# nubot-nudt/RDMNet

Hardware: AMD Instinct MI355X
Metric: scan-pairs/sec (whole node) (higher is better)
Workload: dtype f32

## Files before the change

include/rdmnet_hip.h:

```cpp
#ifndef RDMNET_HIP_H_
#define RDMNET_HIP_H_

#include <stddef.h>
#include <stdint.h>

#ifdef __cplusplus
extern "C" {
#endif

#define RDM_ABI_VERSION 2

int rdm_abi_version(void);
size_t rdm_abi_struct_size(int which);
const char* rdm_last_error(void);

int rdm_rehash_schedule(int64_t max_elems, int64_t* at_host, int64_t* buckets_host, int cap);

size_t rdm_grid_subsample_workspace_bytes(int64_t n_points, int batch);
int rdm_grid_subsample(const float* points, int64_t n_points, const int64_t* lengths, int batch,
                       float voxel_size, float* out_points, int64_t* out_lengths, void* ws,
                       size_t ws_bytes, void* stream);
int rdm_grid_subsample_form(const float* points, int64_t n_points, const int64_t* lengths, int batch, float voxel_size,
                            float* out_points, int64_t* out_lengths, void* ws, size_t ws_bytes, void* stream, int form);

// ... 157 lines not shown
int rdm_row_positive(const float* x, int64_t n, int64_t c, int64_t ld, uint8_t* out, void* stream);

size_t rdm_group_norm_workspace_bytes(int64_t n, int64_t c);
int rdm_group_norm(const float* x, int64_t n, int64_t c, int64_t ldx, int groups, const float* gamma,
                   const float* beta, float eps, const float* residual, int64_t ldr, int act, float* y,
                   int64_t ldy, uint8_t* positive, void* ws, size_t ws_bytes, void* stream);
int rdm_group_norm_form(const float* x, int64_t n, int64_t c, int64_t ldx, int groups, const float* gamma,
                        const float* beta, float eps, const float* residual, int64_t ldr, int act, float* y, int64_t ldy,
                        uint8_t* positive, void* ws, size_t ws_bytes, int form, void* stream);
size_t rdm_linear_group_norm_workspace_bytes(int64_t m, int64_t n);
int rdm_linear_group_norm(const float* x, int64_t ldx, const float* w, int64_t ldw, const float* bias,
                          const float* rowdiv, int64_t m, int64_t n, int64_t k, int groups, const float* gamma,
                          const float* beta, float eps, const float* residual, int64_t ldr, int act, float* lin_out,
                          int64_t ld_lin, float* y, int64_t ldy, uint8_t* positive, void* ws, size_t ws_bytes,
                          void* stream);
int rdm_patch_scores(const float* ref_feats, int64_t ld_ref, int64_t n_ref, const int64_t* ref_idx, const float* src_feats,
                     int64_t ld_src, int64_t n_src, const int64_t* src_idx, int64_t batch, int64_t side, int64_t d,
                     const float* rowdiv, float* scores, void* stream);
size_t rdm_decoder_stage_workspace_bytes(int64_t m, int64_t n, int64_t k);
int rdm_decoder_stage(const float* coarse, int64_t n_coarse, int64_t c1, int64_t ld1, const int64_t* idx, int64_t ldi,
                      const float* skip, int64_t c2, int64_t ld2, int64_t m, const float* w, int64_t ldw, const float* bias,
                      int64_t n, int groups, const float* gamma, const float* beta, float eps, int act, float* lin_out,
                      int64_t ld_lin, float* y, int64_t ldy, void* ws, size_t ws_bytes, void* stream);
int rdm_layer_norm(const float* x, int64_t n, int64_t c, int64_t ldx, const float* residual,
                   int64_t ldr, const float* gamma, const float* beta, float eps, int act, float* y,
                   int64_t ldy, void* stream);
int rdm_linear_layer_norm(const float* x, int64_t ldx, const float* w, int64_t ldw, const float* bias, int64_t m, int64_t n,
                          int64_t k, const float* residual, int64_t ldr, const float* gamma, const float* beta, float eps,
                          int act, float* y, int64_t ldy, void* stream);
int rdm_attention_tail(const float* hidden, int64_t ld_hidden, const float* x, int64_t ldx, int64_t m, int64_t d,
// ... 372 lines not shown
```

rdmnet_amd/_lib.py:

```python
import ctypes
import os

_HERE = os.path.dirname(os.path.abspath(__file__))
LIB_PATH = os.environ.get('RDM_LIB_PATH') or os.path.join(_HERE, 'librdmnet_hip.so')

c_void = ctypes.c_void_p
c_i64 = ctypes.c_int64
c_int = ctypes.c_int
c_f32 = ctypes.c_float
c_size = ctypes.c_size_t

ABI_VERSION = 2


class FineMatchingOptions(ctypes.Structure):
    _fields_ = [('topk', ctypes.c_int32), ('mutual', ctypes.c_int32), ('use_dustbin', ctypes.c_int32),
                ('use_global_score', ctypes.c_int32), ('confidence_threshold', ctypes.c_float),
                ('correspondence_limit', ctypes.c_int32)]

    @classmethod
    def of(cls, topk=1, mutual=False, use_dustbin=True, confidence_threshold=0.0, use_global_score=False,
           correspondence_limit=None):
        return cls(int(topk), int(bool(mutual)), int(bool(use_dustbin)), int(bool(use_global_score)), float(confidence_threshold),
                   0 if correspondence_limit is None else int(correspondence_limit))
# ... 124 lines not shown
    'rdm_pose_graph_pair_covariances_host': (c_int, [c_i64, c_i64, c_void, c_void, c_void, c_i64, c_void, c_void]),
    'rdm_pose_graph_pair_terms_host': (c_int, [c_void, c_void, c_void, c_void, c_void, c_void, c_void, c_void]),
    'rdm_pose_graph_edge_terms_host': (c_int, [c_void, c_void, c_void, c_void, ctypes.c_double, c_int, c_void]),
    'rdm_pose_graph_retract_host': (c_int, [c_void, c_void, c_void]),
    'rdm_neighbor_histogram': (c_int, [c_void, c_i64, c_void, c_int, c_void]),
    'rdm_radius_grid_records': (c_void, [c_void, c_size, c_i64]),
    'rdm_row_positive': (c_int, [c_void, c_i64, c_i64, c_i64, c_void, c_void]),
    'rdm_group_norm_workspace_bytes': (c_size, [c_i64, c_i64]),
    'rdm_group_norm': (c_int, [c_void, c_i64, c_i64, c_i64, c_int, c_void, c_void, c_f32, c_void, c_i64, c_int,
                               c_void, c_i64, c_void, c_void, c_size, c_void]),
    'rdm_group_norm_form': (c_int, [c_void, c_i64, c_i64, c_i64, c_int, c_void, c_void, c_f32, c_void, c_i64, c_int,
                                    c_void, c_i64, c_void, c_void, c_size, c_int, c_void]),
    'rdm_linear_group_norm_workspace_bytes': (c_size, [c_i64, c_i64]),
    'rdm_linear_group_norm': (c_int, [c_void, c_i64, c_void, c_i64, c_void, c_void, c_i64, c_i64, c_i64, c_int, c_void, c_void,
                                      c_f32, c_void, c_i64, c_int, c_void, c_i64, c_void, c_i64, c_void, c_void, c_size, c_void]),
    'rdm_patch_scores': (c_int, [c_void, c_i64, c_i64, c_void, c_void, c_i64, c_i64, c_void, c_i64, c_i64, c_i64, c_void, c_void,
                                 c_void]),
    'rdm_decoder_stage_workspace_bytes': (c_size, [c_i64, c_i64, c_i64]),
    'rdm_decoder_stage': (c_int, [c_void, c_i64, c_i64, c_i64, c_void, c_i64, c_void, c_i64, c_i64, c_i64, c_void, c_i64, c_void,
                                  c_i64, c_int, c_void, c_void, c_f32, c_int, c_void, c_i64, c_void, c_i64, c_void, c_size, c_void]),
    'rdm_layer_norm': (c_int, [c_void, c_i64, c_i64, c_i64, c_void, c_i64, c_void, c_void, c_f32, c_int, c_void,
                               c_i64, c_void]),
    'rdm_linear_layer_norm': (c_int, [c_void, c_i64, c_void, c_i64, c_void, c_i64, c_i64, c_i64, c_void, c_i64, c_void, c_void,
                                      c_f32, c_int, c_void, c_i64, c_void]),
    'rdm_attention_tail': (c_int, [c_void, c_i64, c_void, c_i64, c_i64, c_i64, c_void, c_i64, c_void, c_void, c_void, c_void, c_i64,
                                   c_void, c_void, c_i64, c_void, c_void, c_void, c_f32, c_void, c_i64, c_void]),
    'rdm_attention_tail_packed_floats': (c_size, []),
    'rdm_attention_tail_pack_weights': (c_int, [c_void, c_i64, c_void, c_i64, c_void, c_i64, c_void, c_void]),
    'rdm_attention_tail_packed': (c_int, [c_void, c_i64, c_void, c_i64, c_i64, c_i64, c_void, c_void, c_void, c_void, c_void, c_void,
                                          c_void, c_void, c_f32, c_void, c_i64, c_void]),
# ... 198 lines not shown
```

rdmnet_amd/csrc/engine.hip:

```cpp
#include <algorithm>
#include <cmath>
#include <cstring>
#include <atomic>
#include <chrono>
#include <functional>
#include <map>
#include <memory>
#include <string>
#include <vector>

#include "../../include/rdmnet_hip.h"
#include <ctime>

#include "common.h"
#include "internal.h"
#include "lockstep.h"

namespace {

using namespace rdm;

struct Mat {
  float* p = nullptr;
  int64_t rows = 0, cols = 0, ld = 0;
// ... 226 lines not shown
  lockstep_align();
  rdm_engine* e = r.e;
  const Linear* Lp = lin_param(r, name + ".mlp");
  if (!Lp) return RDM_ERR_ARG;
  const Linear& L = *Lp;
  Mat t = e->mat(x.rows, L.out);
  y = e->mat(x.rows, L.out);
  ENG_ALLOC(t.p); ENG_ALLOC(y.p);
  float *g, *b;
  ENG_CHECK(norm_params(r, name + ".norm.norm", &g, &b));
  return rdm_linear_group_norm(x.p, x.ld, L.b, L.ldb, L.bias, nullptr, x.rows, L.out, L.kpad, r.groups, g, b, 1e-5f,
                               res ? res->p : nullptr, res ? res->ld : 0, act, t.p, t.ld, y.p, y.ld, positive, r.ws,
                               r.ws_bytes, r.st);
}

int decoder_stage(Run& r, const std::string& lin_name, const std::string* norm_name, const Mat& coarse, const int64_t* up_idx,
                  int64_t up_ld, const Mat& skip, int64_t m, Mat& y, int64_t n_cols = 0) {
  lockstep_align();
  rdm_engine* e = r.e;
  const Linear* Lp = lin_param(r, lin_name);
  if (!Lp) return RDM_ERR_ARG;
  const Linear& L = *Lp;
  RDM_REQUIRE(coarse.cols + skip.cols == L.in, "rdm_engine: %s expects %lld input columns", lin_name.c_str(), (long long)L.in);
  RDM_REQUIRE(n_cols >= 0 && n_cols <= L.out && (n_cols == 0 || !norm_name), "rdm_engine: %s cannot compute %lld of its columns",
              lin_name.c_str(), (long long)n_cols);
  const int64_t n = n_cols > 0 ? n_cols : L.out;
  Mat t = e->mat(m, L.out);
  ENG_ALLOC(t.p);
  float *g = nullptr, *b = nullptr;
  if (norm_name) {
// ... 1111 lines not shown
      ENG_CHECK(kpconv(rr, name + ".KPConv", x, enc.x_pos, q, s, t, sigma, name + ".norm", y, order));
    } else {
      Mat h = x;
      uint8_t* h_pos = e->alloc<uint8_t>(x.rows > 0 ? x.rows : 1);
      ENG_ALLOC(h_pos);
      if (e->params->lin.count(name + ".unary1.mlp")) {
        ENG_CHECK(unary(rr, name + ".unary1", x, h, 2, nullptr, h_pos));
      } else {
        ENG_CHECK(rdm_row_positive(x.p, x.rows, x.cols, x.ld, h_pos, rr.st));
      }
      Mat cn;
      Mat sc = x;
      ENG_CHECK(kpconv(rr, name + ".KPConv", h, h_pos, q, s, t, sigma, name + ".norm_conv", cn, order,
                       strided[b] ? &x : nullptr, strided[b] ? &sc : nullptr));
      if (e->params->lin.count(name + ".unary_shortcut.mlp")) {
        Mat s2;
        ENG_CHECK(unary(rr, name + ".unary_shortcut", sc, s2, 0, nullptr, nullptr));
        sc = s2;
      }
      ENG_CHECK(unary(rr, name + ".unary2", cn, y, 2, &sc, nullptr));
    }
    x = y;
    tap(rr, name.c_str(), x);
    if (b % 3 == 1) enc.feats[b / 3] = x;
  }
  enc.blocks = b1;
  return RDM_OK;
}

struct Coarse {
  Mat buf;
  Mat x;
  float* n2p = nullptr;
};

// ... 385 lines not shown
  const rdm_engine_config& c = e->cfg;
  const int64_t n0 = n_ref + n_src;
  Level* lv = py.lv;
  py.flags = e->alloc<int32_t>(64);
  ENG_ALLOC(py.flags);
  bool overlap_l0 = false;
  if (overlap) {
    const auto t_poll = std::chrono::steady_clock::now();
    do {
      overlap_l0 = hipStreamQuery(r.st) == hipSuccess;
    } while (!overlap_l0 && std::chrono::steady_clock::now() - t_poll < std::chrono::microseconds(40));
  }
  Run rs = r;
  if (overlap_l0) {
    rs.st = e->side;
    rs.ws_bytes = std::max<size_t>(size_t(96) << 20, rdm_linear_group_norm_workspace_bytes(n0, 128));
    rs.ws = e->alloc<char>(rs.ws_bytes);
    ENG_ALLOC(rs.ws);
  }
  fill_words<int32_t>(py.flags, 64, 0, overlap_l0 ? rs.st : r.st);
  const bool full = e->keep_taps || e->collate_only;
  lv[0].n = n0; lv[0].n_ref = n_ref;
  lv[0].pts = e->alloc<float>(3 * n0);
  lv[0].lengths = e->alloc<int64_t>(2);
  ENG_ALLOC(lv[0].pts); ENG_ALLOC(lv[0].lengths);
  float* pts0 = lv[0].pts;
  int64_t* len0 = lv[0].lengths;
  if (overlap_l0) {
    pts0 = e->alloc<float>(3 * n0);
    len0 = e->alloc<int64_t>(2);
    ENG_ALLOC(pts0); ENG_ALLOC(len0);
// ... 87 lines not shown
  else if (dd) ENG_CHECK(pyramid_from_data_dict(r, *dd, py));
  else ENG_CHECK(collate_pair(r, overlap, side_guard, ref_points, n_ref, src_points, n_src, py, enc));
  for (int i = 0; i < 5; ++i) {
    res->level_sizes[i] = py.lv[i].n;
    res->level_ref_sizes[i] = py.lv[i].n_ref;
  }
  tap_pyramid(r, py);
  if (e->collate_only) {
    res->arena_used = e->arena_off;
    return RDM_OK;
  }

  {
    size_t need = r.ws_bytes;
    for (int l = 0; l < c.num_stages; ++l)
      need = std::max(need, rdm_linear_group_norm_workspace_bytes(py.lv[l].n, int64_t(128) << l));
    if (need > r.ws_bytes) {
      r.ws_bytes = need;
      r.ws = e->alloc<char>(r.ws_bytes);
      ENG_ALLOC(r.ws);
    }
  }

  if (enc.blocks == 0) ENG_CHECK(encoder_input(r, dd, n0, enc));
  ENG_CHECK(encoder_blocks(r, py, enc.blocks, 14, enc));
  tap(r, "feats_c_enc", enc.feats[4]);
  Coarse co;
  ENG_CHECK(transformer1(r, py, enc.feats[4], co));

  Mat dec;
  const std::function<int()> fork_decoder = [&]() -> int {
// ... 379 lines not shown
```

rdmnet_amd/csrc/gemm.hip:

```cpp
#include "../../include/rdmnet_hip.h"
#include <cmath>
#include <cstdlib>

#include "common.h"
#include "internal.h"
#include "lockstep.h"

namespace {

using namespace rdm;

typedef float f32x16 __attribute__((ext_vector_type(16)));
typedef float f32x4_t __attribute__((ext_vector_type(4)));

struct GemmArgs {
  const float* A = nullptr;
  const float* B = nullptr;
  float* C = nullptr;
  const float* bias = nullptr;
  const float* rowdiv = nullptr;
  int M = 0, N = 0, K = 0;
  int lda = 0, ldb = 0, ldc = 0;
  long long sa = 0, sb = 0, sc = 0;
  int act = 0;
// ... 1113 lines not shown
  char* gws = ar.take<char>(gemm_ws);
  double* partial = ar.take<double>(static_cast<size_t>(gemm_stats_max_blocks(m)) * 2 * n);
  const size_t gn_ws = rdm_group_norm_workspace_bytes(m, n);
  char* nws = ar.take<char>(gn_ws);
  if (!ar.ok) {
    set_error("rdm_linear_group_norm: workspace too small (%zu < %zu)", ws_bytes, ar.off);
    return RDM_ERR_WORKSPACE;
  }
  int nblk = 0;
  if (int e = gemm_with_stats(x, ldx, w, ldw, lin_out, ld_lin, m, n, k, bias, rowdiv, gws, gemm_ws, partial, &nblk, stream))
    return e;
  return group_norm_finish(partial, nblk, lin_out, m, n, ld_lin, groups, gamma, beta, eps, residual, ldr, act, y, ldy,
                           positive, nws, gn_ws, stream);
}

extern "C" int rdm_patch_scores(const float* ref_feats, int64_t ld_ref, int64_t n_ref, const int64_t* ref_idx,
                                const float* src_feats, int64_t ld_src, int64_t n_src, const int64_t* src_idx, int64_t batch,
                                int64_t side, int64_t d, const float* rowdiv, float* scores, void* stream) {
  using namespace rdm;
  RDM_REQUIRE(ref_feats && src_feats && ref_idx && src_idx && scores, "rdm_patch_scores: null pointer");
  RDM_REQUIRE(batch >= 0 && side > 0 && d > 0 && d % 4 == 0 && ld_ref % 4 == 0 && ld_src % 4 == 0 && n_ref > 0 && n_src > 0,
              "rdm_patch_scores: bad sizes");
  RDM_REQUIRE(((reinterpret_cast<uintptr_t>(ref_feats) | reinterpret_cast<uintptr_t>(src_feats)) & 15) == 0,
              "rdm_patch_scores: features must be 16-byte aligned");
  if (batch == 0) return RDM_OK;
  GemmArgs g;
  g.A = ref_feats; g.B = src_feats; g.C = scores; g.rowdiv = rowdiv;
  g.M = static_cast<int>(side); g.N = static_cast<int>(side); g.K = static_cast<int>(d);
  g.lda = static_cast<int>(ld_ref); g.ldb = static_cast<int>(ld_src); g.ldc = static_cast<int>(side);
  g.sc = side * side;
// ... 135 lines not shown
```

rdmnet_amd/csrc/internal.h:

```cpp
#pragma once
#include <cstddef>
#include <cstdint>

namespace rdm {

int gemm_with_stats(const float* a, int64_t lda, const float* b, int64_t ldb, float* c, int64_t ldc, int64_t m,
                    int64_t n, int64_t k, const float* bias, const float* rowdiv, void* ws, size_t ws_bytes,
                    double* gn_partial, int* gn_blocks, void* stream);

void gemm_set_lds_pad(unsigned bytes);
int gemm_concat_with_stats(const float* coarse, int64_t ld1, int64_t c1, int64_t n_coarse, const int64_t* idx, int64_t ldi,
                           const float* skip, int64_t ld2, int64_t c2, const float* b, int64_t ldb, float* c, int64_t ldc,
                           int64_t m, int64_t n, int64_t n_need, const float* bias, int act, float* pbuf, size_t pbuf_floats,
                           void* ws, size_t ws_bytes, double* gn_partial, int* gn_blocks, void* stream);
int decoder_stage_cols(const float* coarse, int64_t n_coarse, int64_t c1, int64_t ld1, const int64_t* idx, int64_t ldi,
                       const float* skip, int64_t c2, int64_t ld2, int64_t m, const float* w, int64_t ldw, const float* bias,
                       int64_t n, int64_t n_need, int groups, const float* gamma, const float* beta, float eps, int act,
                       float* lin_out, int64_t ld_lin, float* y, int64_t ldy, void* ws, size_t ws_bytes, void* stream);

int gemm_pair(const float* a0, int64_t lda0, const float* b0, int64_t ldb0, float* c0, int64_t ldc0, int64_t m0, int64_t n0,
              int64_t k0, const float* bias0, const float* a1, int64_t lda1, const float* b1, int64_t ldb1, float* c1,
              int64_t ldc1, int64_t m1, int64_t n1, int64_t k1, const float* bias1, void* ws, size_t ws_bytes, void* stream);

inline int64_t gemm_stats_max_blocks(int64_t m) { return (m + 7) / 8 + 1; }

int grid_subsample_mode(const float* points, int64_t n_points, const int64_t* lengths, int batch, float voxel_size,
                        float* out_points, int64_t* out_lengths, void* ws, size_t ws_bytes, void* stream, int mode);

int group_norm_finish(const double* partial, int nblk, const float* x, int64_t n, int64_t c, int64_t ldx, int groups,
                      const float* gamma, const float* beta, float eps, const float* residual, int64_t ldr, int act,
                      float* y, int64_t ldy, uint8_t* positive, void* ws, size_t ws_bytes, void* stream, int form = 0);

int gather_rows_multi(int n, const void* const* x, const int64_t* n_src, const int64_t* words, const int64_t* ldx,
                      const int64_t* const* idx, const int64_t* m, void* const* y, const int64_t* ldy, void* stream);

int radius_grid_build_multi(int n, const float* const* s_points, const int64_t* n_s, const int64_t* const* s_lengths, int batch,
                            const float* radius, void* const* grid_ws, const size_t* grid_ws_bytes, void* stream);

int radius_grid_build_trivial(const float* s_points, int64_t n_s, const int64_t* s_lengths, int batch, void* grid_ws,
                              size_t grid_ws_bytes, void* stream);

int compact_indices_pair(const uint8_t* keep, int64_t n_ref, int64_t n, int32_t* order, int32_t* counts,
                         const int32_t* mirror_src, int32_t* mirror_dst, int mirror_words, void* stream);

int gather_max_ordered(const float* x, int64_t n_s, int64_t c, int64_t ldx, const int64_t* idx, int64_t m, int64_t h, int64_t ldi,
                       const int32_t* width, float* y, int64_t ldy, const float* order_records, int i32, void* stream);
// ... 24 lines not shown
```

rdmnet_amd/csrc/norm.hip:

```cpp
#include "../../include/rdmnet_hip.h"
#include "common.h"
#include "internal.h"
#include "lockstep.h"

namespace {

using namespace rdm;

constexpr int kGnRowsPerBlock = 64;

__device__ __forceinline__ void gn_partial_kernel_body(const dim3 blockIdx, const dim3 gridDim, const float* x, int n, int c, int ld,
                                                         double* partial) {
  (void)blockIdx; (void)gridDim;
  __shared__ double red[2][256];
  const int r0 = blockIdx.x * kGnRowsPerBlock;
  const int r1 = min(n, r0 + kGnRowsPerBlock);
  const int cw = c < 256 ? c : 256;
  const int lanes = 256 / cw;
  const int col_in = threadIdx.x % cw, rl = threadIdx.x / cw;
  const int col = blockIdx.y * 256 + col_in;
  double s = 0.0, ss = 0.0;
  if (rl < lanes && col < c)
    for (int r = r0 + rl; r < r1; r += lanes) {
      const double v = x[static_cast<int64_t>(r) * ld + col];
// ... 88 lines not shown
    for (int blk = 0; blk < nblk; ++blk) {
      a += partial[(static_cast<int64_t>(blk) * 2 + 0) * c + k];
      b += partial[(static_cast<int64_t>(blk) * 2 + 1) * c + k];
    }
    gs += a;
    gss += b;
  }
  const double cnt = static_cast<double>(n) * cpg;
  const double mean = gs / cnt;
  double var = gss / cnt - mean * mean;
  if (var < 0.0) var = 0.0;
  const double gsc = 1.0 / sqrt(var + static_cast<double>(eps)) * static_cast<double>(gamma[col]);
  scale[col] = static_cast<float>(gsc);
  shift[col] = static_cast<float>(static_cast<double>(beta[col]) - mean * gsc);
}
template <int COLS>
__device__ __forceinline__ void gn_finalize_kernel_body(const dim3 blockIdx, const dim3 gridDim, const double* partial, int nblk, int n,
                                                            int c, int groups, const float* gamma,
                                                            const float* beta, float eps, float* scale,
                                                            float* shift) {
  (void)blockIdx; (void)gridDim;
  __shared__ GnFinalizeLds<COLS> L;
  const float2 v = gn_scale_shift<COLS>(L, blockIdx.x * COLS, partial, nblk, n, c, groups, gamma, beta, eps);
  const int col = blockIdx.x * COLS + threadIdx.x % COLS;
  if (threadIdx.x / COLS == 0 && col < c) {
    scale[col] = v.x;
    shift[col] = v.y;
  }
}


constexpr int kGnFusedRows = 256;
__device__ __forceinline__ void gn_finalize_apply_kernel_body(const dim3 blockIdx, const dim3 gridDim, const double* partial, int nblk, const float* x, int n, int c, int ldx,
                                                                  int groups, const float* gamma, const float* beta, float eps,
                                                                  const float* res, int ldr, int act, float* y, int ldy) {
  (void)blockIdx; (void)gridDim;
  __shared__ GnFinalizeLds<64> L;
  __shared__ float sc_l[64], sh_l[64];
  const int col0 = blockIdx.x * 64;
  const float2 v = gn_scale_shift<64>(L, col0, partial, nblk, n, c, groups, gamma, beta, eps);
  if (threadIdx.x < 64) {
    sc_l[threadIdx.x] = v.x;
    sh_l[threadIdx.x] = v.y;
  }
  __syncthreads();
  const int q = threadIdx.x & 15, rl = threadIdx.x >> 4;
  const int col = col0 + 4 * q;
  if (col >= c) return;
  const float4 sc = *reinterpret_cast<const float4*>(sc_l + 4 * q), sh = *reinterpret_cast<const float4*>(sh_l + 4 * q);
  const int r1 = min(n, (static_cast<int>(blockIdx.y) + 1) * kGnFusedRows);
  for (int row = blockIdx.y * kGnFusedRows + rl; row < r1; row += 64) {
    const float4 xv = *reinterpret_cast<const float4*>(x + static_cast<int64_t>(row) * ldx + col);
    float o[4] = {__builtin_fmaf(xv.x, sc.x, sh.x), __builtin_fmaf(xv.y, sc.y, sh.y), __builtin_fmaf(xv.z, sc.z, sh.z),
                  __builtin_fmaf(xv.w, sc.w, sh.w)};
    if (res) {
      const float4 rv = *reinterpret_cast<const float4*>(res + static_cast<int64_t>(row) * ldr + col);
      o[0] += rv.x; o[1] += rv.y; o[2] += rv.z; o[3] += rv.w;
    }
#pragma unroll
    for (int k = 0; k < 4; ++k) {
      if (act == 2) o[k] = o[k] > 0.f ? o[k] : 0.1f * o[k];
      else if (act == 1) o[k] = o[k] > 0.f ? o[k] : 0.f;
    }
    *reinterpret_cast<float4*>(y + static_cast<int64_t>(row) * ldy + col) = make_float4(o[0], o[1], o[2], o[3]);
  }
}


__device__ __forceinline__ void gn_apply_kernel_body(const dim3 blockIdx, const dim3 gridDim, const float* x, int n, int c, int ldx,
                                                       const float* scale, const float* shift,
                                                       const float* res, int ldr, int act, float* y,
                                                       int ldy, unsigned char* positive) {
  (void)blockIdx; (void)gridDim;
  const int row = blockIdx.x * 4 + (threadIdx.x >> 6);
  if (row >= n) return;
  const int lane = threadIdx.x & 63;
  float rs = 0.f;
  for (int col = lane; col < c; col += 64) {
    float v = x[static_cast<int64_t>(row) * ldx + col] * scale[col] + shift[col];
    if (res) v += res[static_cast<int64_t>(row) * ldr + col];
    if (act == 2) v = v > 0.f ? v : 0.1f * v;
    else if (act == 1) v = v > 0.f ? v : 0.f;
    y[static_cast<int64_t>(row) * ldy + col] = v;
    rs += v;
  }
  if (positive) {
    rs = wave_sum(rs);
    if (lane == 0) positive[row] = rs > 0.f ? 1 : 0;
  }
}


__device__ __forceinline__ void gn_apply_wide_kernel_body(const dim3 blockIdx, const dim3 gridDim, const float* x, int n, int c4, int ldx, const float* scale,
                                                            const float* shift, const float* res, int ldr, int act,
                                                            float* y, int ldy, unsigned char* positive) {
  (void)blockIdx; (void)gridDim;
  const int64_t t = blockIdx.x * 256ll + threadIdx.x;
  const bool live = t < static_cast<int64_t>(n) * c4;
  if (!live && !positive) return;
  float rs4[4] = {0.f, 0.f, 0.f, 0.f};
  const int row = live ? static_cast<int>(t / c4) : 0, col = live ? static_cast<int>(t % c4) * 4 : 0;
  if (live) {
  const float4 xv = *reinterpret_cast<const float4*>(x + static_cast<int64_t>(row) * ldx + col);
  const float4 sc = *reinterpret_cast<const float4*>(scale + col), sh = *reinterpret_cast<const float4*>(shift + col);
  float v[4] = {__builtin_fmaf(xv.x, sc.x, sh.x), __builtin_fmaf(xv.y, sc.y, sh.y), __builtin_fmaf(xv.z, sc.z, sh.z),
                __builtin_fmaf(xv.w, sc.w, sh.w)};
  if (res) {
    const float4 rv = *reinterpret_cast<const float4*>(res + static_cast<int64_t>(row) * ldr + col);
    v[0] += rv.x; v[1] += rv.y; v[2] += rv.z; v[3] += rv.w;
  }
#pragma unroll
  for (int k = 0; k < 4; ++k) {
    if (act == 2) v[k] = v[k] > 0.f ? v[k] : 0.1f * v[k];
    else if (act == 1) v[k] = v[k] > 0.f ? v[k] : 0.f;
  }
  *reinterpret_cast<float4*>(y + static_cast<int64_t>(row) * ldy + col) = make_float4(v[0], v[1], v[2], v[3]);
#pragma unroll
  for (int k = 0; k < 4; ++k) rs4[k] = v[k];
  }
  if (positive) {
    for (int o = c4 >> 1; o > 0; o >>= 1)
#pragma unroll
      for (int k = 0; k < 4; ++k) rs4[k] += __shfl_xor(rs4[k], o, 64);
// ... 211 lines not shown
                     static_cast<uint32_t*>(y), static_cast<int>(ldy));
  else if (threads == 128) ::rdm::launch<gather_rows_kernel_body, 128>(dim3(static_cast<unsigned>(m)), 0, static_cast<hipStream_t>(stream), static_cast<const uint32_t*>(x), static_cast<int>(n_src),
                     static_cast<int>(words), static_cast<int>(ldx), idx, static_cast<int>(m),
                     static_cast<uint32_t*>(y), static_cast<int>(ldy));
  else ::rdm::launch<gather_rows_kernel_body, 64>(dim3(static_cast<unsigned>(m)), 0, static_cast<hipStream_t>(stream), static_cast<const uint32_t*>(x), static_cast<int>(n_src),
                     static_cast<int>(words), static_cast<int>(ldx), idx, static_cast<int>(m),
                     static_cast<uint32_t*>(y), static_cast<int>(ldy));
  return launch_status("gather_rows_kernel");
}

extern "C" size_t rdm_group_norm_workspace_bytes(int64_t n, int64_t c) {
  const size_t nblk = static_cast<size_t>(rdm::ceil_div<int64_t>(n > 0 ? n : 1, kGnRowsPerBlock));
  return rdm::align_up(nblk * 2 * c * sizeof(double)) + rdm::align_up(2 * c * sizeof(float));
}

int rdm::group_norm_finish(const double* partial_in, int nblk, const float* x, int64_t n, int64_t c, int64_t ldx,
                           int groups, const float* gamma, const float* beta, float eps, const float* residual,
                           int64_t ldr, int act, float* y, int64_t ldy, uint8_t* positive, void* ws, size_t ws_bytes,
                           void* stream, int form) {
  Arena ar(ws, ws_bytes);
  const int own_blk = static_cast<int>(ceil_div<int64_t>(n, kGnRowsPerBlock));
  double* partial = ar.take<double>(static_cast<size_t>(own_blk) * 2 * c);
  float* ss = ar.take<float>(2 * c);
  if (!ar.ok) {
    set_error("rdm_group_norm: workspace too small (%zu < %zu)", ws_bytes, ar.off);
    return RDM_ERR_WORKSPACE;
  }
  hipStream_t st = static_cast<hipStream_t>(stream);
  const double* use = partial_in;
  if (nblk <= 0) {
    ::rdm::launch<gn_partial_kernel_body, 256>(dim3(own_blk, ceil_div<int64_t>(c, 256)), 0, st, x,
                       static_cast<int>(n), static_cast<int>(c), static_cast<int>(ldx), partial);
    use = partial;
    nblk = own_blk;
  }
  const bool vec_ok = c % 4 == 0 && ldx % 4 == 0 && ldy % 4 == 0 && (!residual || ldr % 4 == 0) &&
                      (reinterpret_cast<uintptr_t>(x) & 15) == 0 && (reinterpret_cast<uintptr_t>(y) & 15) == 0 &&
                      (!residual || (reinterpret_cast<uintptr_t>(residual) & 15) == 0);
  static const bool fin64 = ::rdm::dev_knob("RDM_GN_FINALIZE_64") != nullptr;
  const bool narrow = !fin64 && nblk >= 128 && c / groups <= 16 && 16 % (c / groups) == 0;
  const bool whole_groups = 64 % (c / groups) == 0;
  if (form != 1 && !narrow && !positive && vec_ok && c % 64 == 0 && n <= 4096 && whole_groups) {
    RDM_DUP_LOOP("gnfin")
    ::rdm::launch<gn_finalize_apply_kernel_body, 1024>(dim3(static_cast<unsigned>(c / 64), static_cast<unsigned>(ceil_div<int64_t>(n, kGnFusedRows))), 0, st, use, nblk, x, static_cast<int>(n), static_cast<int>(c), static_cast<int>(ldx), groups, gamma, beta,
                       eps, residual, static_cast<int>(ldr), act, y, static_cast<int>(ldy));
    return launch_status("gn_finalize_apply_kernel");
  }
  {
    RDM_DUP_LOOP("gnfin")
    if (!whole_groups)
      ::rdm::launch<gn_finalize_any_width_kernel_body, 256>(dim3(ceil_div<int64_t>(c, 256)), 0, st, use, nblk,
                         static_cast<int>(n), static_cast<int>(c), groups, gamma, beta, eps, ss, ss + c);
    else if (narrow)
      ::rdm::launch<gn_finalize_kernel_body<16>, 1024>(dim3(ceil_div<int64_t>(c, 16)), 0, st, use, nblk,
                         static_cast<int>(n), static_cast<int>(c), groups, gamma, beta, eps, ss, ss + c);
    else
    ::rdm::launch<gn_finalize_kernel_body<64>, 1024>(dim3(ceil_div<int64_t>(c, 64)), 0, st, use, nblk,
                       static_cast<int>(n), static_cast<int>(c), groups, gamma, beta, eps, ss, ss + c);
  }
  static const bool narrow_rows = ::rdm::dev_knob("RDM_GN_APPLY_ROWS") != nullptr;
  const int64_t c4 = c / 4;
  const bool flag_ok = c4 == 8 || c4 == 16 || c4 == 32;
  const bool wide = vec_ok && (narrow_rows ? (!positive && c >= 256) : (!positive || flag_ok));
  RDM_DUP_LOOP("gnapply")
  if (wide)
    ::rdm::launch<gn_apply_wide_kernel_body, 256>(dim3(ceil_div<int64_t>(n * (c / 4), 256)), 0, st, x, static_cast<int>(n),
                       static_cast<int>(c / 4), static_cast<int>(ldx), ss, ss + c, residual, static_cast<int>(ldr), act, y,
                       static_cast<int>(ldy), positive);
  else
    ::rdm::launch<gn_apply_kernel_body, 256>(dim3(ceil_div<int64_t>(n, 4)), 0, st, x,
                       static_cast<int>(n), static_cast<int>(c), static_cast<int>(ldx), ss, ss + c, residual,
                       static_cast<int>(ldr), act, y, static_cast<int>(ldy), positive);
  return launch_status("group_norm kernels");
}

extern "C" int rdm_group_norm(const float* x, int64_t n, int64_t c, int64_t ldx, int groups,
                              const float* gamma, const float* beta, float eps, const float* residual,
                              int64_t ldr, int act, float* y, int64_t ldy, uint8_t* positive, void* ws,
                              size_t ws_bytes, void* stream) {
  using namespace rdm;
  RDM_REQUIRE(x && gamma && beta && y, "rdm_group_norm: null pointer");
  RDM_REQUIRE(n >= 0 && c > 0 && groups > 0 && c % groups == 0 && c <= 4096 && 64 % (c / groups) == 0,
              "rdm_group_norm: bad sizes (n=%lld c=%lld groups=%d)", (long long)n, (long long)c, groups);
  if (n == 0) return RDM_OK;
  return group_norm_finish(nullptr, 0, x, n, c, ldx, groups, gamma, beta, eps, residual, ldr, act, y, ldy, positive, ws,
                           ws_bytes, stream);
}

// ... 106 lines not shown
```

rdmnet_amd/ops.py:

```python
import ctypes
import numbers

import torch

from . import _lib, config

ACT_NONE, ACT_RELU, ACT_LEAKY = 0, 1, 2


def pad4(n):
    return (int(n) + 3) // 4 * 4


class Scratch:

    def __init__(self, device):
        self.device = device
        self.buf = torch.empty(1 << 24, dtype=torch.uint8, device=device)

    def get(self, nbytes):
        if self.buf.numel() < nbytes:
            self.buf = torch.empty(int(nbytes * 1.25) + 256, dtype=torch.uint8, device=self.device)
        return self.buf

# ... 141 lines not shown

def linear_group_norm(x, b, k, n, bias, gamma, beta, groups, *, rowdiv=None, act=ACT_NONE, residual=None,
                      want_positive=False, eps=1e-5):
    L = _lib.lib()
    m = x.shape[0]
    lin = feat_empty(m, n, x.device)
    y = feat_empty(m, n, x.device)
    pos = torch.empty((max(m, 1),), dtype=torch.uint8, device=x.device) if want_positive else None
    ws = scratch(x.device, L.rdm_linear_group_norm_workspace_bytes(m, n))
    _lib.check(L.rdm_linear_group_norm(x.data_ptr(), _ld(x), b.data_ptr(), _ld(b), _lib.ptr(bias), _lib.ptr(rowdiv), m, n, k,
                                       groups, gamma.data_ptr(), beta.data_ptr(), eps, _lib.ptr(residual),
                                       _ld(residual) if residual is not None else 0, act, lin.data_ptr(), _ld(lin),
                                       y.data_ptr(), _ld(y), _lib.ptr(pos), ws.data_ptr(), ws.numel(), _lib.stream_ptr()),
               'rdm_linear_group_norm')
    return (y, pos) if want_positive else y


def decoder_stage(coarse, idx, skip, b, n, bias, gamma=None, beta=None, groups=32, *, act=ACT_NONE, eps=1e-5):
    L = _lib.lib()
    m, c1, c2 = skip.shape[0], coarse.shape[1], skip.shape[1]
    lin = feat_empty(m, n, skip.device)
    y = feat_empty(m, n, skip.device) if gamma is not None else None
    ws = scratch(skip.device, L.rdm_decoder_stage_workspace_bytes(m, n, c1 + c2))
    _lib.check(L.rdm_decoder_stage(coarse.data_ptr(), coarse.shape[0], c1, _ld(coarse), idx.data_ptr(), _ld(idx), skip.data_ptr(),
                                   c2, _ld(skip), m, b.data_ptr(), _ld(b), _lib.ptr(bias), n, groups, _lib.ptr(gamma),
                                   _lib.ptr(beta), eps, act, lin.data_ptr(), _ld(lin), _lib.ptr(y), _ld(y) if y is not None else 0,
                                   ws.data_ptr(), ws.numel(), _lib.stream_ptr()), 'rdm_decoder_stage')
    return y if gamma is not None else lin


# ... 1867 lines not shown
```

Before: 625.1.

## Fuse shortcut unary group-norm into the residual block's final group-norm apply

In strided residual blocks, the shortcut unary (linear + group norm) used to be run as its own pass and its output then added as the residual of unary2. Now both GEMMs emit partial statistics, and one finalize/apply pass normalises the shortcut product on the fly while adding it to unary2's normalised output. Finalize kernels take a second stat set through blockIdx.y. This removes a separate group-norm finalize and apply pass plus one full write and read of the intermediate, at the cost of extra branching and a larger workspace.

```diff
diff --git a/include/rdmnet_hip.h b/include/rdmnet_hip.h
--- a/include/rdmnet_hip.h
+++ b/include/rdmnet_hip.h
@@ -195,6 +195,12 @@
                           const float* beta, float eps, const float* residual, int64_t ldr, int act, float* lin_out,
                           int64_t ld_lin, float* y, int64_t ldy, uint8_t* positive, void* ws, size_t ws_bytes,
                           void* stream);
+size_t rdm_linear_group_norm_pair_workspace_bytes(int64_t m, int64_t n);
+int rdm_linear_group_norm_pair(const float* x, int64_t ldx, const float* w, int64_t ldw, const float* bias, int64_t k,
+                               const float* xs, int64_t ldxs, const float* w_s, int64_t ldws, const float* bias_s, int64_t ks,
+                               int64_t m, int64_t n, int groups, const float* gamma, const float* beta, const float* gamma_s,
+                               const float* beta_s, float eps, int act, float* lin_out, int64_t ld_lin, float* lin_out_s,
+                               int64_t ld_lin_s, float* y, int64_t ldy, void* ws, size_t ws_bytes, void* stream);
 int rdm_patch_scores(const float* ref_feats, int64_t ld_ref, int64_t n_ref, const int64_t* ref_idx, const float* src_feats,
                      int64_t ld_src, int64_t n_src, const int64_t* src_idx, int64_t batch, int64_t side, int64_t d,
                      const float* rowdiv, float* scores, void* stream);
diff --git a/rdmnet_amd/_lib.py b/rdmnet_amd/_lib.py
--- a/rdmnet_amd/_lib.py
+++ b/rdmnet_amd/_lib.py
@@ -162,6 +162,10 @@
     'rdm_linear_group_norm_workspace_bytes': (c_size, [c_i64, c_i64]),
     'rdm_linear_group_norm': (c_int, [c_void, c_i64, c_void, c_i64, c_void, c_void, c_i64, c_i64, c_i64, c_int, c_void, c_void,
                                       c_f32, c_void, c_i64, c_int, c_void, c_i64, c_void, c_i64, c_void, c_void, c_size, c_void]),
+    'rdm_linear_group_norm_pair_workspace_bytes': (c_size, [c_i64, c_i64]),
+    'rdm_linear_group_norm_pair': (c_int, [c_void, c_i64, c_void, c_i64, c_void, c_i64, c_void, c_i64, c_void, c_i64, c_void, c_i64,
+                                           c_i64, c_i64, c_int, c_void, c_void, c_void, c_void, c_f32, c_int, c_void, c_i64, c_void,
+                                           c_i64, c_void, c_i64, c_void, c_size, c_void]),
     'rdm_patch_scores': (c_int, [c_void, c_i64, c_i64, c_void, c_void, c_i64, c_i64, c_void, c_i64, c_i64, c_i64, c_void, c_void,
                                  c_void]),
     'rdm_decoder_stage_workspace_bytes': (c_size, [c_i64, c_i64, c_i64]),
diff --git a/rdmnet_amd/csrc/engine.hip b/rdmnet_amd/csrc/engine.hip
--- a/rdmnet_amd/csrc/engine.hip
+++ b/rdmnet_amd/csrc/engine.hip
@@ -264,6 +264,39 @@
                                r.ws_bytes, r.st);
 }
 
+int unary_with_shortcut(Run& r, const std::string& name, const Mat& x, const std::string& sc_name, const Mat& sc, Mat& y) {
+  lockstep_align();
+  rdm_engine* e = r.e;
+  const Linear* Lp = lin_param(r, name + ".mlp");
+  const Linear* Sp = Lp ? lin_param(r, sc_name + ".mlp") : nullptr;
+  if (!Lp || !Sp) return RDM_ERR_ARG;
+  const Linear &L = *Lp, &S = *Sp;
+  RDM_REQUIRE(L.out == S.out && x.rows == sc.rows, "rdm_engine: %s and %s disagree in shape", name.c_str(), sc_name.c_str());
+  const int64_t m = x.rows, n = L.out;
+  Mat t = e->mat(m, n), ts = e->mat(m, n);
+  y = e->mat(m, n);
+  ENG_ALLOC(t.p); ENG_ALLOC(ts.p); ENG_ALLOC(y.p);
+  float *g, *b, *gs, *bs;
+  ENG_CHECK(norm_params(r, name + ".norm.norm", &g, &b));
+  ENG_CHECK(norm_params(r, sc_name + ".norm.norm", &gs, &bs));
+  if (m == 0) return RDM_OK;
+  const size_t gemm_ws = rdm_gemm_workspace_bytes(m, n, 1);
+  const size_t stat_bytes = align_up(static_cast<size_t>(gemm_stats_max_blocks(m)) * 2 * n * sizeof(double));
+  const size_t gn_ws = group_norm_residual_norm_workspace_bytes(m, n);
+  RDM_REQUIRE(gemm_ws + 2 * stat_bytes + gn_ws <= r.ws_bytes, "rdm_engine: scratch too small");
+  char* base = static_cast<char*>(r.ws);
+  double* part = reinterpret_cast<double*>(base + gemm_ws);
+  double* part_s = reinterpret_cast<double*>(base + gemm_ws + stat_bytes);
+  int nblk = 0, nblk_s = 0;
+  ENG_CHECK(gemm_with_stats(sc.p, sc.ld, S.b, S.ldb, ts.p, ts.ld, m, n, S.kpad, S.bias, nullptr, r.ws, gemm_ws, part_s, &nblk_s, r.st));
+  lockstep_align();
+  ENG_CHECK(gemm_with_stats(x.p, x.ld, L.b, L.ldb, t.p, t.ld, m, n, L.kpad, L.bias, nullptr, r.ws, gemm_ws, part, &nblk, r.st));
+  lockstep_align();
+  const GnResidualNorm rn{part_s, nblk_s, gs, bs};
+  return group_norm_finish_residual_norm(part, nblk, t.p, m, n, t.ld, r.groups, g, b, 1e-5f, ts.p, ts.ld, rn, 2, y.p, y.ld,
+                                         base + gemm_ws + 2 * stat_bytes, gn_ws, r.st);
+}
+
 int decoder_stage(Run& r, const std::string& lin_name, const std::string* norm_name, const Mat& coarse, const int64_t* up_idx,
                   int64_t up_ld, const Mat& skip, int64_t m, Mat& y, int64_t n_cols = 0) {
   lockstep_align();
@@ -1405,11 +1438,10 @@
       ENG_CHECK(kpconv(rr, name + ".KPConv", h, h_pos, q, s, t, sigma, name + ".norm_conv", cn, order,
                        strided[b] ? &x : nullptr, strided[b] ? &sc : nullptr));
       if (e->params->lin.count(name + ".unary_shortcut.mlp")) {
-        Mat s2;
-        ENG_CHECK(unary(rr, name + ".unary_shortcut", sc, s2, 0, nullptr, nullptr));
-        sc = s2;
+        ENG_CHECK(unary_with_shortcut(rr, name + ".unary2", cn, name + ".unary_shortcut", sc, y));
+      } else {
+        ENG_CHECK(unary(rr, name + ".unary2", cn, y, 2, &sc, nullptr));
       }
-      ENG_CHECK(unary(rr, name + ".unary2", cn, y, 2, &sc, nullptr));
     }
     x = y;
     tap(rr, name.c_str(), x);
@@ -1825,7 +1857,7 @@
   Run rs = r;
   if (overlap_l0) {
     rs.st = e->side;
-    rs.ws_bytes = std::max<size_t>(size_t(96) << 20, rdm_linear_group_norm_workspace_bytes(n0, 128));
+    rs.ws_bytes = std::max<size_t>(size_t(96) << 20, rdm_linear_group_norm_pair_workspace_bytes(n0, 128));
     rs.ws = e->alloc<char>(rs.ws_bytes);
     ENG_ALLOC(rs.ws);
   }
@@ -1943,7 +1975,7 @@
   {
     size_t need = r.ws_bytes;
     for (int l = 0; l < c.num_stages; ++l)
-      need = std::max(need, rdm_linear_group_norm_workspace_bytes(py.lv[l].n, int64_t(128) << l));
+      need = std::max(need, rdm_linear_group_norm_pair_workspace_bytes(py.lv[l].n, int64_t(128) << l));
     if (need > r.ws_bytes) {
       r.ws_bytes = need;
       r.ws = e->alloc<char>(r.ws_bytes);
diff --git a/rdmnet_amd/csrc/gemm.hip b/rdmnet_amd/csrc/gemm.hip
--- a/rdmnet_amd/csrc/gemm.hip
+++ b/rdmnet_amd/csrc/gemm.hip
@@ -1151,6 +1151,46 @@
                            positive, nws, gn_ws, stream);
 }
 
+extern "C" size_t rdm_linear_group_norm_pair_workspace_bytes(int64_t m, int64_t n) {
+  return rdm_gemm_workspace_bytes(m, n, 1) + 2 * rdm::align_up(static_cast<size_t>(rdm::gemm_stats_max_blocks(m)) * 2 * n * sizeof(double)) +
+         rdm::group_norm_residual_norm_workspace_bytes(m, n) + 1024;
+}
+
+extern "C" int rdm_linear_group_norm_pair(const float* x, int64_t ldx, const float* w, int64_t ldw, const float* bias, int64_t k,
+                                          const float* xs, int64_t ldxs, const float* w_s, int64_t ldws, const float* bias_s,
+                                          int64_t ks, int64_t m, int64_t n, int groups, const float* gamma, const float* beta,
+                                          const float* gamma_s, const float* beta_s, float eps, int act, float* lin_out,
+                                          int64_t ld_lin, float* lin_out_s, int64_t ld_lin_s, float* y, int64_t ldy, void* ws,
+                                          size_t ws_bytes, void* stream) {
+  using namespace rdm;
+  RDM_REQUIRE(x && w && xs && w_s && gamma && beta && gamma_s && beta_s && lin_out && lin_out_s && y,
+              "rdm_linear_group_norm_pair: null pointer");
+  RDM_REQUIRE(k % 4 == 0 && ldx % 4 == 0 && ldw % 4 == 0 && ks % 4 == 0 && ldxs % 4 == 0 && ldws % 4 == 0,
+              "rdm_linear_group_norm_pair: K, ldx, ldw of both products must be multiples of 4");
+  RDM_REQUIRE(m >= 0 && n > 0 && groups > 0 && n % groups == 0 && n <= 4096 && 64 % (n / groups) == 0,
+              "rdm_linear_group_norm_pair: bad sizes (m=%lld n=%lld groups=%d)", (long long)m, (long long)n, groups);
+  if (m == 0) return RDM_OK;
+  Arena ar(ws, ws_bytes);
+  const size_t gemm_ws = rdm_gemm_workspace_bytes(m, n, 1);
+  char* gws = ar.take<char>(gemm_ws);
+  double* partial = ar.take<double>(static_cast<size_t>(gemm_stats_max_blocks(m)) * 2 * n);
+  double* partial_s = ar.take<double>(static_cast<size_t>(gemm_stats_max_blocks(m)) * 2 * n);
+  const size_t gn_ws = group_norm_residual_norm_workspace_bytes(m, n);
+  char* nws = ar.take<char>(gn_ws);
+  if (!ar.ok) {
+    set_error("rdm_linear_group_norm_pair: workspace too small (%zu < %zu)", ws_bytes, ar.off);
+    return RDM_ERR_WORKSPACE;
+  }
+  int nblk = 0, nblk_s = 0;
+  if (int e = gemm_with_stats(xs, ldxs, w_s, ldws, lin_out_s, ld_lin_s, m, n, ks, bias_s, nullptr, gws, gemm_ws, partial_s, &nblk_s,
+                              stream))
+    return e;
+  if (int e = gemm_with_stats(x, ldx, w, ldw, lin_out, ld_lin, m, n, k, bias, nullptr, gws, gemm_ws, partial, &nblk, stream)) return e;
+  const GnResidualNorm rn{partial_s, nblk_s, gamma_s, beta_s};
+  return group_norm_finish_residual_norm(partial, nblk, lin_out, m, n, ld_lin, groups, gamma, beta, eps, lin_out_s, ld_lin_s, rn, act,
+                                         y, ldy, nws, gn_ws, stream);
+}
+
 extern "C" int rdm_patch_scores(const float* ref_feats, int64_t ld_ref, int64_t n_ref, const int64_t* ref_idx,
                                 const float* src_feats, int64_t ld_src, int64_t n_src, const int64_t* src_idx, int64_t batch,
                                 int64_t side, int64_t d, const float* rowdiv, float* scores, void* stream) {
diff --git a/rdmnet_amd/csrc/internal.h b/rdmnet_amd/csrc/internal.h
--- a/rdmnet_amd/csrc/internal.h
+++ b/rdmnet_amd/csrc/internal.h
@@ -30,6 +30,18 @@
 int group_norm_finish(const double* partial, int nblk, const float* x, int64_t n, int64_t c, int64_t ldx, int groups,
                       const float* gamma, const float* beta, float eps, const float* residual, int64_t ldr, int act,
                       float* y, int64_t ldy, uint8_t* positive, void* ws, size_t ws_bytes, void* stream, int form = 0);
+
+struct GnResidualNorm {
+  const double* partial;
+  int nblk;
+  const float* gamma;
+  const float* beta;
+};
+size_t group_norm_residual_norm_workspace_bytes(int64_t n, int64_t c);
+int group_norm_finish_residual_norm(const double* partial, int nblk, const float* x, int64_t n, int64_t c, int64_t ldx, int groups,
+                                    const float* gamma, const float* beta, float eps, const float* residual, int64_t ldr,
+                                    const GnResidualNorm& rn, int act, float* y, int64_t ldy, void* ws, size_t ws_bytes,
+                                    void* stream);
 
 int gather_rows_multi(int n, const void* const* x, const int64_t* n_src, const int64_t* words, const int64_t* ldx,
                       const int64_t* const* idx, const int64_t* m, void* const* y, const int64_t* ldy, void* stream);
diff --git a/rdmnet_amd/csrc/norm.hip b/rdmnet_amd/csrc/norm.hip
--- a/rdmnet_amd/csrc/norm.hip
+++ b/rdmnet_amd/csrc/norm.hip
@@ -126,13 +126,26 @@
   scale[col] = static_cast<float>(gsc);
   shift[col] = static_cast<float>(static_cast<double>(beta[col]) - mean * gsc);
 }
+struct GnStatSet {
+  const double* partial;
+  int nblk;
+  const float* gamma;
+  const float* beta;
+  float* scale;
+  float* shift;
+};
 template <int COLS>
-__device__ __forceinline__ void gn_finalize_kernel_body(const dim3 blockIdx, const dim3 gridDim, const double* partial, int nblk, int n,
-                                                            int c, int groups, const float* gamma,
-                                                            const float* beta, float eps, float* scale,
-                                                            float* shift) {
+__device__ __forceinline__ void gn_finalize_kernel_body(const dim3 blockIdx, const dim3 gridDim, GnStatSet s0, GnStatSet s1, int n, int c,
+                                                            int groups, float eps) {
   (void)blockIdx; (void)gridDim;
   __shared__ GnFinalizeLds<COLS> L;
+  const bool second = blockIdx.y != 0;
+  const double* partial = second ? s1.partial : s0.partial;
+  const int nblk = second ? s1.nblk : s0.nblk;
+  const float* gamma = second ? s1.gamma : s0.gamma;
+  const float* beta = second ? s1.beta : s0.beta;
+  float* scale = second ? s1.scale : s0.scale;
+  float* shift = second ? s1.shift : s0.shift;
   const float2 v = gn_scale_shift<COLS>(L, blockIdx.x * COLS, partial, nblk, n, c, groups, gamma, beta, eps);
   const int col = blockIdx.x * COLS + threadIdx.x % COLS;
   if (threadIdx.x / COLS == 0 && col < c) {
@@ -145,10 +158,12 @@
 constexpr int kGnFusedRows = 256;
 __device__ __forceinline__ void gn_finalize_apply_kernel_body(const dim3 blockIdx, const dim3 gridDim, const double* partial, int nblk, const float* x, int n, int c, int ldx,
                                                                   int groups, const float* gamma, const float* beta, float eps,
-                                                                  const float* res, int ldr, int act, float* y, int ldy) {
+                                                                  const float* res, int ldr, int act, float* y, int ldy,
+                                                                  const double* partial_r, int nblk_r, const float* gamma_r,
+                                                                  const float* beta_r) {
   (void)blockIdx; (void)gridDim;
   __shared__ GnFinalizeLds<64> L;
-  __shared__ float sc_l[64], sh_l[64];
+  __shared__ float sc_l[64], sh_l[64], scr_l[64], shr_l[64];
   const int col0 = blockIdx.x * 64;
   const float2 v = gn_scale_shift<64>(L, col0, partial, nblk, n, c, groups, gamma, beta, eps);
   if (threadIdx.x < 64) {
@@ -156,17 +171,33 @@
     sh_l[threadIdx.x] = v.y;
   }
   __syncthreads();
+  if (partial_r) {
+    const float2 w = gn_scale_shift<64>(L, col0, partial_r, nblk_r, n, c, groups, gamma_r, beta_r, eps);
+    if (threadIdx.x < 64) {
+      scr_l[threadIdx.x] = w.x;
+      shr_l[threadIdx.x] = w.y;
+    }
+    __syncthreads();
+  }
   const int q = threadIdx.x & 15, rl = threadIdx.x >> 4;
   const int col = col0 + 4 * q;
   if (col >= c) return;
   const float4 sc = *reinterpret_cast<const float4*>(sc_l + 4 * q), sh = *reinterpret_cast<const float4*>(sh_l + 4 * q);
+  float4 scr = make_float4(0.f, 0.f, 0.f, 0.f), shr = scr;
+  if (partial_r) {
+    scr = *reinterpret_cast<const float4*>(scr_l + 4 * q);
+    shr = *reinterpret_cast<const float4*>(shr_l + 4 * q);
+  }
   const int r1 = min(n, (static_cast<int>(blockIdx.y) + 1) * kGnFusedRows);
   for (int row = blockIdx.y * kGnFusedRows + rl; row < r1; row += 64) {
     const float4 xv = *reinterpret_cast<const float4*>(x + static_cast<int64_t>(row) * ldx + col);
     float o[4] = {__builtin_fmaf(xv.x, sc.x, sh.x), __builtin_fmaf(xv.y, sc.y, sh.y), __builtin_fmaf(xv.z, sc.z, sh.z),
                   __builtin_fmaf(xv.w, sc.w, sh.w)};
     if (res) {
-      const float4 rv = *reinterpret_cast<const float4*>(res + static_cast<int64_t>(row) * ldr + col);
+      float4 rv = *reinterpret_cast<const float4*>(res + static_cast<int64_t>(row) * ldr + col);
+      if (partial_r)
+        rv = make_float4(__builtin_fmaf(rv.x, scr.x, shr.x), __builtin_fmaf(rv.y, scr.y, shr.y), __builtin_fmaf(rv.z, scr.z, shr.z),
+                         __builtin_fmaf(rv.w, scr.w, shr.w));
       o[0] += rv.x; o[1] += rv.y; o[2] += rv.z; o[3] += rv.w;
     }
 #pragma unroll
@@ -182,7 +213,8 @@
 __device__ __forceinline__ void gn_apply_kernel_body(const dim3 blockIdx, const dim3 gridDim, const float* x, int n, int c, int ldx,
                                                        const float* scale, const float* shift,
                                                        const float* res, int ldr, int act, float* y,
-                                                       int ldy, unsigned char* positive) {
+                                                       int ldy, unsigned char* positive, const float* scale_r,
+                                                       const float* shift_r) {
   (void)blockIdx; (void)gridDim;
   const int row = blockIdx.x * 4 + (threadIdx.x >> 6);
   if (row >= n) return;
@@ -190,7 +222,11 @@
   float rs = 0.f;
   for (int col = lane; col < c; col += 64) {
     float v = x[static_cast<int64_t>(row) * ldx + col] * scale[col] + shift[col];
-    if (res) v += res[static_cast<int64_t>(row) * ldr + col];
+    if (res) {
+      float rv = res[static_cast<int64_t>(row) * ldr + col];
+      if (scale_r) rv = __builtin_fmaf(rv, scale_r[col], shift_r[col]);
+      v += rv;
+    }
     if (act == 2) v = v > 0.f ? v : 0.1f * v;
     else if (act == 1) v = v > 0.f ? v : 0.f;
     y[static_cast<int64_t>(row) * ldy + col] = v;
@@ -205,7 +241,8 @@
 
 __device__ __forceinline__ void gn_apply_wide_kernel_body(const dim3 blockIdx, const dim3 gridDim, const float* x, int n, int c4, int ldx, const float* scale,
                                                             const float* shift, const float* res, int ldr, int act,
-                                                            float* y, int ldy, unsigned char* positive) {
+                                                            float* y, int ldy, unsigned char* positive, const float* scale_r,
+                                                            const float* shift_r) {
   (void)blockIdx; (void)gridDim;
   const int64_t t = blockIdx.x * 256ll + threadIdx.x;
   const bool live = t < static_cast<int64_t>(n) * c4;
@@ -218,7 +255,12 @@
   float v[4] = {__builtin_fmaf(xv.x, sc.x, sh.x), __builtin_fmaf(xv.y, sc.y, sh.y), __builtin_fmaf(xv.z, sc.z, sh.z),
                 __builtin_fmaf(xv.w, sc.w, sh.w)};
   if (res) {
-    const float4 rv = *reinterpret_cast<const float4*>(res + static_cast<int64_t>(row) * ldr + col);
+    float4 rv = *reinterpret_cast<const float4*>(res + static_cast<int64_t>(row) * ldr + col);
+    if (scale_r) {
+      const float4 scr = *reinterpret_cast<const float4*>(scale_r + col), shr = *reinterpret_cast<const float4*>(shift_r + col);
+      rv = make_float4(__builtin_fmaf(rv.x, scr.x, shr.x), __builtin_fmaf(rv.y, scr.y, shr.y), __builtin_fmaf(rv.z, scr.z, shr.z),
+                       __builtin_fmaf(rv.w, scr.w, shr.w));
+    }
     v[0] += rv.x; v[1] += rv.y; v[2] += rv.z; v[3] += rv.w;
   }
 #pragma unroll
@@ -460,14 +502,18 @@
   return rdm::align_up(nblk * 2 * c * sizeof(double)) + rdm::align_up(2 * c * sizeof(float));
 }
 
-int rdm::group_norm_finish(const double* partial_in, int nblk, const float* x, int64_t n, int64_t c, int64_t ldx,
-                           int groups, const float* gamma, const float* beta, float eps, const float* residual,
-                           int64_t ldr, int act, float* y, int64_t ldy, uint8_t* positive, void* ws, size_t ws_bytes,
+namespace {
+
+int group_norm_finish_impl(const double* partial_in, int nblk, const float* x, int64_t n, int64_t c, int64_t ldx, int groups,
+                           const float* gamma, const float* beta, float eps, const float* residual, int64_t ldr,
+                           const GnResidualNorm* rn, int act, float* y, int64_t ldy, uint8_t* positive, void* ws, size_t ws_bytes,
                            void* stream, int form) {
   Arena ar(ws, ws_bytes);
   const int own_blk = static_cast<int>(ceil_div<int64_t>(n, kGnRowsPerBlock));
   double* partial = ar.take<double>(static_cast<size_t>(own_blk) * 2 * c);
   float* ss = ar.take<float>(2 * c);
+  double* partial_r = rn ? ar.take<double>(static_cast<size_t>(own_blk) * 2 * c) : nullptr;
+  float* ss_r = rn ? ar.take<float>(2 * c) : nullptr;
   if (!ar.ok) {
     set_error("rdm_group_norm: workspace too small (%zu < %zu)", ws_bytes, ar.off);
     return RDM_ERR_WORKSPACE;
@@ -480,44 +526,88 @@
     use = partial;
     nblk = own_blk;
   }
+  const double* use_r = rn ? rn->partial : nullptr;
+  int nblk_r = rn ? rn->nblk : 0;
+  if (rn && nblk_r <= 0) {
+    ::rdm::launch<gn_partial_kernel_body, 256>(dim3(own_blk, ceil_div<int64_t>(c, 256)), 0, st, residual,
+                       static_cast<int>(n), static_cast<int>(c), static_cast<int>(ldr), partial_r);
+    use_r = partial_r;
+    nblk_r = own_blk;
+  }
   const bool vec_ok = c % 4 == 0 && ldx % 4 == 0 && ldy % 4 == 0 && (!residual || ldr % 4 == 0) &&
                       (reinterpret_cast<uintptr_t>(x) & 15) == 0 && (reinterpret_cast<uintptr_t>(y) & 15) == 0 &&
                       (!residual || (reinterpret_cast<uintptr_t>(residual) & 15) == 0);
   static const bool fin64 = ::rdm::dev_knob("RDM_GN_FINALIZE_64") != nullptr;
-  const bool narrow = !fin64 && nblk >= 128 && c / groups <= 16 && 16 % (c / groups) == 0;
+  const bool narrow_cols = !fin64 && c / groups <= 16 && 16 % (c / groups) == 0;
+  const bool narrow = narrow_cols && nblk >= 128, narrow_r = rn && narrow_cols && nblk_r >= 128;
   const bool whole_groups = 64 % (c / groups) == 0;
-  if (form != 1 && !narrow && !positive && vec_ok && c % 64 == 0 && n <= 4096 && whole_groups) {
+  if (form != 1 && !narrow && !narrow_r && !positive && vec_ok && c % 64 == 0 && n <= 4096 && whole_groups) {
     RDM_DUP_LOOP("gnfin")
     ::rdm::launch<gn_finalize_apply_kernel_body, 1024>(dim3(static_cast<unsigned>(c / 64), static_cast<unsigned>(ceil_div<int64_t>(n, kGnFusedRows))), 0, st, use, nblk, x, static_cast<int>(n), static_cast<int>(c), static_cast<int>(ldx), groups, gamma, beta,
-                       eps, residual, static_cast<int>(ldr), act, y, static_cast<int>(ldy));
+                       eps, residual, static_cast<int>(ldr), act, y, static_cast<int>(ldy), use_r, nblk_r,
+                       rn ? rn->gamma : nullptr, rn ? rn->beta : nullptr);
     return launch_status("gn_finalize_apply_kernel");
   }
   {
+    const GnStatSet s0{use, nblk, gamma, beta, ss, ss + c};
+    const GnStatSet s1 = rn ? GnStatSet{use_r, nblk_r, rn->gamma, rn->beta, ss_r, ss_r + c} : GnStatSet{nullptr, 0, nullptr, nullptr, nullptr, nullptr};
+    const int ni = static_cast<int>(n), ci = static_cast<int>(c);
     RDM_DUP_LOOP("gnfin")
-    if (!whole_groups)
-      ::rdm::launch<gn_finalize_any_width_kernel_body, 256>(dim3(ceil_div<int64_t>(c, 256)), 0, st, use, nblk,
-                         static_cast<int>(n), static_cast<int>(c), groups, gamma, beta, eps, ss, ss + c);
-    else if (narrow)
-      ::rdm::launch<gn_finalize_kernel_body<16>, 1024>(dim3(ceil_div<int64_t>(c, 16)), 0, st, use, nblk,
-                         static_cast<int>(n), static_cast<int>(c), groups, gamma, beta, eps, ss, ss + c);
-    else
-    ::rdm::launch<gn_finalize_kernel_body<64>, 1024>(dim3(ceil_div<int64_t>(c, 64)), 0, st, use, nblk,
-                       static_cast<int>(n), static_cast<int>(c), groups, gamma, beta, eps, ss, ss + c);
+    if (!whole_groups) {
+      ::rdm::launch<gn_finalize_any_width_kernel_body, 256>(dim3(ceil_div<int64_t>(c, 256)), 0, st, use, nblk, ni, ci, groups, gamma,
+                                                            beta, eps, ss, ss + c);
+      if (rn)
+        ::rdm::launch<gn_finalize_any_width_kernel_body, 256>(dim3(ceil_div<int64_t>(c, 256)), 0, st, use_r, nblk_r, ni, ci, groups,
+                                                              rn->gamma, rn->beta, eps, ss_r, ss_r + c);
+    } else if (rn && narrow != narrow_r) {
+      const GnStatSet none{nullptr, 0, nullptr, nullptr, nullptr, nullptr};
+      if (narrow) ::rdm::launch<gn_finalize_kernel_body<16>, 1024>(dim3(ceil_div<int64_t>(c, 16), 1), 0, st, s0, none, ni, ci, groups, eps);
+      else ::rdm::launch<gn_finalize_kernel_body<64>, 1024>(dim3(ceil_div<int64_t>(c, 64), 1), 0, st, s0, none, ni, ci, groups, eps);
+      if (narrow_r) ::rdm::launch<gn_finalize_kernel_body<16>, 1024>(dim3(ceil_div<int64_t>(c, 16), 1), 0, st, s1, none, ni, ci, groups, eps);
+      else ::rdm::launch<gn_finalize_kernel_body<64>, 1024>(dim3(ceil_div<int64_t>(c, 64), 1), 0, st, s1, none, ni, ci, groups, eps);
+    } else if (narrow) {
+      ::rdm::launch<gn_finalize_kernel_body<16>, 1024>(dim3(ceil_div<int64_t>(c, 16), rn ? 2 : 1), 0, st, s0, s1, ni, ci, groups, eps);
+    } else {
+      ::rdm::launch<gn_finalize_kernel_body<64>, 1024>(dim3(ceil_div<int64_t>(c, 64), rn ? 2 : 1), 0, st, s0, s1, ni, ci, groups, eps);
+    }
   }
   static const bool narrow_rows = ::rdm::dev_knob("RDM_GN_APPLY_ROWS") != nullptr;
   const int64_t c4 = c / 4;
   const bool flag_ok = c4 == 8 || c4 == 16 || c4 == 32;
   const bool wide = vec_ok && (narrow_rows ? (!positive && c >= 256) : (!positive || flag_ok));
+  const float* scale_r = rn ? ss_r : nullptr;
+  const float* shift_r = rn ? ss_r + c : nullptr;
   RDM_DUP_LOOP("gnapply")
   if (wide)
     ::rdm::launch<gn_apply_wide_kernel_body, 256>(dim3(ceil_div<int64_t>(n * (c / 4), 256)), 0, st, x, static_cast<int>(n),
                        static_cast<int>(c / 4), static_cast<int>(ldx), ss, ss + c, residual, static_cast<int>(ldr), act, y,
-                       static_cast<int>(ldy), positive);
+                       static_cast<int>(ldy), positive, scale_r, shift_r);
   else
     ::rdm::launch<gn_apply_kernel_body, 256>(dim3(ceil_div<int64_t>(n, 4)), 0, st, x,
                        static_cast<int>(n), static_cast<int>(c), static_cast<int>(ldx), ss, ss + c, residual,
-                       static_cast<int>(ldr), act, y, static_cast<int>(ldy), positive);
+                       static_cast<int>(ldr), act, y, static_cast<int>(ldy), positive, scale_r, shift_r);
   return launch_status("group_norm kernels");
+}
+
+}
+
+int rdm::group_norm_finish(const double* partial_in, int nblk, const float* x, int64_t n, int64_t c, int64_t ldx,
+                           int groups, const float* gamma, const float* beta, float eps, const float* residual,
+                           int64_t ldr, int act, float* y, int64_t ldy, uint8_t* positive, void* ws, size_t ws_bytes,
+                           void* stream, int form) {
+  return group_norm_finish_impl(partial_in, nblk, x, n, c, ldx, groups, gamma, beta, eps, residual, ldr, nullptr, act, y, ldy,
+                                positive, ws, ws_bytes, stream, form);
+}
+
+size_t rdm::group_norm_residual_norm_workspace_bytes(int64_t n, int64_t c) { return 2 * rdm_group_norm_workspace_bytes(n, c); }
+
+int rdm::group_norm_finish_residual_norm(const double* partial, int nblk, const float* x, int64_t n, int64_t c, int64_t ldx,
+                                         int groups, const float* gamma, const float* beta, float eps, const float* residual,
+                                         int64_t ldr, const GnResidualNorm& rn, int act, float* y, int64_t ldy, void* ws,
+                                         size_t ws_bytes, void* stream) {
+  RDM_REQUIRE(residual && rn.gamma && rn.beta, "group_norm: the normalised residual needs its matrix, gamma and beta");
+  return group_norm_finish_impl(partial, nblk, x, n, c, ldx, groups, gamma, beta, eps, residual, ldr, &rn, act, y, ldy, nullptr, ws,
+                                ws_bytes, stream, 0);
 }
 
 extern "C" int rdm_group_norm(const float* x, int64_t n, int64_t c, int64_t ldx, int groups,
diff --git a/rdmnet_amd/ops.py b/rdmnet_amd/ops.py
--- a/rdmnet_amd/ops.py
+++ b/rdmnet_amd/ops.py
@@ -179,6 +179,20 @@
                                        y.data_ptr(), _ld(y), _lib.ptr(pos), ws.data_ptr(), ws.numel(), _lib.stream_ptr()),
                'rdm_linear_group_norm')
     return (y, pos) if want_positive else y
+
+
+def linear_group_norm_pair(x, b, k, xs, bs, ks, n, bias, bias_s, gamma, beta, gamma_s, beta_s, groups, *, act=ACT_LEAKY, eps=1e-5,
+                           return_products=False):
+    L = _lib.lib()
+    m = x.shape[0]
+    lin, lin_s, y = feat_empty(m, n, x.device), feat_empty(m, n, x.device), feat_empty(m, n, x.device)
+    ws = scratch(x.device, L.rdm_linear_group_norm_pair_workspace_bytes(m, n))
+    _lib.check(L.rdm_linear_group_norm_pair(x.data_ptr(), _ld(x), b.data_ptr(), _ld(b), _lib.ptr(bias), k, xs.data_ptr(), _ld(xs),
+                                            bs.data_ptr(), _ld(bs), _lib.ptr(bias_s), ks, m, n, groups, gamma.data_ptr(),
+                                            beta.data_ptr(), gamma_s.data_ptr(), beta_s.data_ptr(), eps, act, lin.data_ptr(),
+                                            _ld(lin), lin_s.data_ptr(), _ld(lin_s), y.data_ptr(), _ld(y), ws.data_ptr(),
+                                            ws.numel(), _lib.stream_ptr()), 'rdm_linear_group_norm_pair')
+    return (y, lin, lin_s) if return_products else y
 
 
 def decoder_stage(coarse, idx, skip, b, n, bias, gamma=None, beta=None, groups=32, *, act=ACT_NONE, eps=1e-5):
```

Measured after the change: 613.8. -1.8%, worse.
